# Da1yuqin/TCDiff

Hardware: AMD Instinct MI355X
Metric: sampled clips/sec (3 dancers x 150 frames, 1000 DDPM steps) (higher is better)
Workload: dtype bf16; 1 GPU; batch=16 clips/GPU, 3 dancers x 150 frames, 1000 DDPM steps (p_sample_loop, CFG w=2, cosine schedule), bf16, 1xMI355X; clips_per_gpu=16, ddpm_steps=1000

## Files before the change

include/tcdiff_hip.h:

```cpp
#ifndef TCDIFF_HIP_H
#define TCDIFF_HIP_H

#include <stdint.h>

#ifdef __cplusplus
extern "C" {
#endif

#ifndef __HIP__
typedef struct ihipStream_t* hipStream_t;
#endif

#define TCDIFF_OK 0
#define TCDIFF_ERR_ARG (-1)
#define TCDIFF_ERR_ALIGN (-2)
#define TCDIFF_ERR_LAUNCH (-3)
#define TCDIFF_ERR_UNSUPPORTED (-4)

#define TC_DTYPE_F32 0
#define TC_DTYPE_BF16 1
#define TC_DTYPE_BF16X3 2

#define TC_ACT_NONE 0
#define TC_ACT_RELU 1
// ... 246 lines not shown
} tcdiff_ct_desc;
int tcdiff_ct_desc_init(int dtype, tcdiff_ct_desc* d);
int tcdiff_cast_transpose_multi(int dtype, const tcdiff_ct_desc* descs_dev, int n_desc, int n_tiles, hipStream_t stream);

typedef struct tcdiff_ws_desc {
    const float* src;
    void* dst;
    long sn, sk;
    int N, K;
    int np_dst, p0, kst_dst, ks0;
} tcdiff_ws_desc;
int tcdiff_pack_row_streams(const tcdiff_ws_desc* descs_dev, int n_desc, int max_elems, hipStream_t stream);
int tcdiff_gemm_rows(const void* A, const void* A2, int split_n, const void* wstream, int M, int N, int K, int lda,
                     const tcdiff_tile_epi* epi, int mt, hipStream_t stream);

int tcdiff_gemm_splitk(int dtype, const void* A, const void* W, int M, int N, int K, int lda, int ldw, float* out,
                       int ldc, int splits, hipStream_t stream);

int tcdiff_gemm_tn(int dtype, const void* A, const void* B, int M, int N, int K, int lda, int ldb, float* out, int ldc,
                   int splits, hipStream_t stream);

#define TC_TN_MAX_PROB 16
typedef struct {
    const void* A; const void* B; float* out;
    int M, N, K, lda, ldb, ldc;
    int nk, unit0;
} tcdiff_tn_problem;
typedef struct {
    int n_prob, total_units, units_per_wg, kc;
    tcdiff_tn_problem p[TC_TN_MAX_PROB];
// ... 210 lines not shown
```

tcdiff_amd/_lib.py:

```python
import ctypes as C
import os

HERE = os.path.dirname(os.path.abspath(__file__))
LIB_PATH = os.environ.get("TCDIFF_LIB_PATH") or os.path.join(HERE, "libtcdiff_gfx950.so")

DT_F32, DT_BF16, DT_BF16X3 = 0, 1, 2
ACT_NONE, ACT_RELU, ACT_GELU, ACT_MISH, ACT_SILU = 0, 1, 2, 3, 4
EPI_STORE_T, EPI_STORE_F32, EPI_QKV_HEADS = 0, 1, 2
ROW_BIAS, ROW_LN_POST, ROW_FILM, ROW_RES, ROW_STORE_X, ROW_NEXT_LN, ROW_STORE_H, ROW_STORE_ROT = \
    1, 2, 4, 8, 16, 32, 64, 128
SAMPLER_DDPM, SAMPLER_DDIM = 0, 1
EXPORT_NORMAL, EXPORT_LONG = 0, 1
SAMPLER_ADVANCE = 0x100
CHAIN_A, CHAIN_B, CHAIN_B_LAST, CHAIN_FULL, CHAIN_FULL_LAST, CHAIN_FRONT = 0, 1, 2, 3, 4, 5

_vp, _i, _f, _l = C.c_void_p, C.c_int, C.c_float, C.c_long


class TileEpi(C.Structure):
    _fields_ = [("mode", _i), ("act", _i), ("scale_q", _f), ("bias", _vp), ("out", _vp), ("out_k", _vp),
                ("out_v", _vp), ("ldc", _i), ("L", _i), ("Lp", _i), ("H", _i), ("n_q", _i), ("n_k", _i),
                ("tok_off", _i), ("seq_off", _i), ("k_splits", _i), ("out2", _vp), ("ldc2", _i), ("act_src", _vp),
                ("ld_src", _i), ("act2", _i), ("drop_seed", _vp), ("drop_site", _i), ("drop_thr", C.c_uint32),
                ("drop_scale", _f), ("hgroup", _i), ("hgroup_stride", _l), ("small_m", _i)]
# ... 110 lines not shown
    "tcdiff_step_prologue": [_i, _vp, _vp],
    "tcdiff_sampler_update": [_i, _vp, _vp, _i, _vp, _vp, _vp, _vp, _i, _i, _i, _vp, _vp, _vp, C.c_uint64, _i, _vp],
    "tcdiff_window_couple": [_vp, _i, _i, _i, _vp],
    "tcdiff_window_couple_step": [_vp, _i, _i, _i, _vp, _vp, _vp],
    "tcdiff_sampler_constrain": [_i, _vp, _vp, _i, _vp, _vp, _i, _i, _i, _vp, _vp, _vp, C.c_uint64, _i, _vp],
    "tcdiff_ema_update": [_vp, _i, _f, _f, _vp],
    "tcdiff_cfg_combine": [_vp, _vp, _i, _f, _vp, _i, _i, _vp],
    "tcdiff_cast_transpose": [_i, _i, _vp, _i, _i, _i, _vp, _i, _i, _vp, _i, _i, _vp, _vp],
    "tcdiff_gemm_splitk": [_i, _vp, _vp, _i, _i, _i, _i, _i, _vp, _i, _i, _vp],
    "tcdiff_gemm_tn": [_i, _vp, _vp, _i, _i, _i, _i, _i, _vp, _i, _i, _vp],
    "tcdiff_gemm_tn_grouped": [_i, C.POINTER(TnProblem), _i, _vp],
    "tcdiff_ct_desc_init": [_i, C.POINTER(CtDesc)],
    "tcdiff_cast_transpose_multi": [_i, _vp, _i, _i, _vp],
    "tcdiff_pack_row_streams": [_vp, _i, _i, _vp],
    "tcdiff_gemm_rows": [_vp, _vp, _i, _vp, _i, _i, _i, _i, _vp, _i, _vp],
    "tcdiff_pos_drop": [_vp, _i, _i, _vp, _i, _vp, _i, C.c_uint32, _f, _vp],
    "tcdiff_act_drop": [_i, _i, _vp, _i, _vp, _i, _i, _i, _i, _vp, _i, C.c_uint32, _f, _vp],
    "tcdiff_act_drop_bwd": [_i, _i, _vp, _i, _vp, _i, _vp, _i, _i, _i, _vp, _i, C.c_uint32, _f, _vp],
    "tcdiff_row_fwd": [_i, C.POINTER(RowArgs), _vp],
    "tcdiff_row_bwd": [_i, C.POINTER(RowArgs), _vp],
    "tcdiff_row_param_reduce": [_vp, _i, _vp, _vp, _vp, _vp, _vp, _vp],
    "tcdiff_attention_train": [_i, _vp, _vp, _vp, _vp, _vp, _vp, _i, _i, _i, _i, _i, _i, _i, _vp, _i, C.c_uint32, _f, _vp],
    "tcdiff_attention_bwd": [_i, _vp, _vp, _vp, _vp, _vp, _vp, _vp, _vp, _vp, _i, _vp, _vp, _i, _i, _i, _i, _i, _i, _i, _i,
                             _f, _vp, _i, C.c_uint32, _f, _vp],
    "tcdiff_add_rows": [_vp, _i, _vp, _i, _vp, _i, _i, _i, _vp],
    "tcdiff_select_rows": [_vp, _vp, _vp, _vp, _i, _l, _vp],
    "tcdiff_select_rows_bwd": [_vp, _vp, _vp, _vp, _i, _l, _vp],
    "tcdiff_pool_bwd": [_vp, _vp, _vp, _i, _i, _i, _vp],
    "tcdiff_loss_total": [_vp, _i, _vp, _vp],
    "tcdiff_loss_terms_bwd": [_vp, _vp, _vp, _vp, _vp, _vp, _vp, _vp, _vp, _i, _i, _i, _i, _i, _vp],
# ... 71 lines not shown
```

tcdiff_amd/build.py:

```python
import os
import subprocess
import sys

HERE = os.path.dirname(os.path.abspath(__file__))
ROOT = os.path.dirname(HERE)
SRC = [os.path.join(HERE, "csrc", f) for f in ("gemm.hip", "attention.hip", "ops.hip", "chain.hip", "train.hip", "train_ops.hip",
                                               "attention_train.hip", "gemm_rows.hip", "chain_split.hip", "export.hip", "navigator.hip", "navigator_train.hip", "navigator_step.hip",
                                               "ingest.hip", "handoff.hip")]
HDR = sorted(os.path.join(HERE, "csrc", h) for h in os.listdir(os.path.join(HERE, "csrc")) if h.endswith(".h")) + \
    [os.path.join(ROOT, "include", "tcdiff_hip.h")]
LIB = os.path.join(HERE, "libtcdiff_gfx950.so")


def needs_build() -> bool:
    if not os.path.exists(LIB):
        return True
    t = os.path.getmtime(LIB)
    return any(os.path.getmtime(f) > t for f in SRC + HDR)


def build(force: bool = False, verbose: bool = True) -> str:
    if not force and not needs_build():
        return LIB
    hipcc = os.environ.get("HIPCC", "/opt/rocm/bin/hipcc")
# ... 24 lines not shown
```

tcdiff_amd/csrc/chain_core.h:

```cpp
#pragma once
#include "common.h"
#include "tcdiff_hip.h"

#define CH_FILM 0
#define CH_VEC 8192
#define CH_SCR 20480
#define CH_ABUF 28672
#define CH_H1C 94208
#define CH_ABUF2 94208
#define CH_STG7 159744
#define CH_SMEM 163840
#define CH_D 4
#define CH_STAGE 4096
#ifndef CH_D8
#define CH_D8 4
#endif
template <int NT> struct ChW {
    static constexpr int NW = 32 / NT;
    static constexpr int D = NT == 8 ? CH_D8 : CH_D;
    static constexpr int STAGE = 1024 * NT;
};

typedef const float* fptr;

// ... 447 lines not shown
            const int row = row0 + 8 * k;
            const u32x4 v = *reinterpret_cast<const u32x4*>(stg + row * 128 + ((ch ^ ((row >> 1) & 7)) << 4));
            if (m < M) *reinterpret_cast<u32x4*>(dst) = v;
            m += 8;
            tokf += 8;
            dst += 8 * 64 * dn;
            if (tokf >= Lf) {
                tokf -= Lf;
                dst += wrap;
            }
        }
    }
    }
}

#define CH_LOG2E 1.4426950408889634f
#ifndef CH_ATT_THR
#define CH_ATT_THR 5.0f
#endif

DEVINL float max3n(float a, float b, float c) { return __builtin_fmaximum_numf(__builtin_fmaximum_numf(a, b), c); }
DEVINL float lane_max8(const f32x4_t& a, const f32x4_t& b, float floor) {
    return max3n(max3n(max3n(max3n(a[0], a[1], a[2]), a[3], b[0]), b[1], b[2]), b[3], floor);
}

template <int MT>
DEVINL void store_qfrag(const f32x4_t (&acc)[4][MT], void* base, float scale, int lblk, int wave, int lane) {
    u32x4* dst = reinterpret_cast<u32x4*>(base) + ((long)(lblk * 8 + wave) * 8) * 64 + lane;
    scale *= CH_LOG2E;
#pragma unroll
// ... 62 lines not shown
```

tcdiff_amd/csrc/gemm_rows.hip:

```cpp
#include "chain_core.h"
#include "train_common.h"

struct RowsArgs {
    const char* A;
    const char* A2;
    const char* wstream;
    int split_n, n_stages, M, N, lda_bytes;
    tcdiff_tile_epi e;
};

DEVINL void unpack8(const u32x4& c, float (&v)[8]) {
#pragma unroll
    for (int i = 0; i < 4; ++i) {
        v[2 * i] = __builtin_bit_cast(float, c[i] << 16);
        v[2 * i + 1] = __builtin_bit_cast(float, c[i] & 0xFFFF0000u);
    }
}
DEVINL u32x4 pack8(const float (&v)[8]) {
    u32x4 c;
#pragma unroll
    for (int i = 0; i < 4; ++i) c[i] = pack_bf2(v[2 * i], v[2 * i + 1]);
    return c;
}

template <int MT, class F>
DEVINL void staged_rows(const f32x4_t (&acc)[4][MT], char* stg, int lane, F&& sink) {
    lane = fresh_v(lane);
    const int c = lane & 15, g = lane >> 4;
    const int row0 = lane >> 3, ch = lane & 7;
    constexpr int NH = MT == 4 ? 2 : 1, NML = MT == 1 ? 1 : 2;
#pragma unroll
    for (int hf = 0; hf < NH; ++hf) {
#pragma unroll
        for (int ml = 0; ml < NML; ++ml) {
            const int rl = 16 * ml + c;
#pragma unroll
            for (int nt = 0; nt < 4; ++nt) {
                const f32x4_t v = acc[nt][2 * hf + ml];
                uint2 pk;
                pk.x = pack_bf2(v[0], v[1]);
                pk.y = pack_bf2(v[2], v[3]);
                *reinterpret_cast<uint2*>(stg + rl * 128 + (((2 * nt + (g >> 1)) ^ ((rl >> 1) & 7)) << 4) + 8 * (g & 1)) = pk;
            }
        }
#pragma unroll
        for (int k = 0; k < 2 * NML; ++k) {
            const int row = row0 + 8 * k;
            const u32x4 v = *reinterpret_cast<const u32x4*>(stg + row * 128 + ((ch ^ ((row >> 1) & 7)) << 4));
            sink(32 * hf + row, ch, v);
        }
    }
}

template <int KST, int MT>
__global__ __launch_bounds__(512) void gemm_rows_kernel(RowsArgs a) {
    constexpr int BR = 16 * MT;
    extern __shared__ __attribute__((aligned(16))) char smem[];
    const int tid = threadIdx.x, lane = tid & 63;
    const int wave = __builtin_amdgcn_readfirstlane(tid >> 6);
    const int m0 = xcd_remap(blockIdx.x, gridDim.x) * BR;
    const int M = a.M;
    char* abuf = smem + CH_ABUF;
    char* abuf2 = smem + CH_ABUF2;
    const bool two = KST == 16 && a.A2 != nullptr;

    if (wave < 2 * MT) {
// ... 221 lines not shown
```

tcdiff_amd/csrc/ops.hip:

```cpp
#include "common.h"
#include "tcdiff_hip.h"

DEVINL long kf_index(int key, int d) {
    const int kt = key >> 5, k32 = key & 31, d32 = d & 31;
    const int g = (d32 & 15) >> 2, jj = 4 * (d32 >> 4) + (d32 & 3);
    return ((long)((kt * 2 + (k32 >> 4)) * 2 + (d >> 5)) * 64 + g * 16 + (k32 & 15)) * 8 + jj;
}
DEVINL long vf_index(int key, int d) {
    const int kt = key >> 5, k32 = key & 31;
    const int g = (k32 & 15) >> 2, jj = 4 * (k32 >> 4) + (k32 & 3);
    return ((long)(kt * 4 + (d >> 4)) * 64 + g * 16 + (d & 15)) * 8 + jj;
}

template <class P>
__global__ __launch_bounds__(256) void ln_rot_kernel(const float* __restrict__ x, int rows, const float* __restrict__ g,
                                                     const float* __restrict__ b, float eps, void* __restrict__ hout,
                                                     void* __restrict__ rout, float* __restrict__ y32,
                                                     const float* __restrict__ rope, int pos_mod, int pos_base) {
    typedef typename P::elem_t T;
    const int lane = threadIdx.x & 63;
    const int row = blockIdx.x * 4 + (threadIdx.x >> 6);
    if (row >= rows) return;
    const float* xr = x + (long)row * 512;
    f32x4_t v[2];
// ... 256 lines not shown
    hipLaunchKernelGGL(step_end_kernel, dim3(1), dim3(64), 0, stream, counter);
    TC_CHECK_LAUNCH();
    return TC_OK;
}

template <class P>
__global__ __launch_bounds__(256) void step_prologue_kernel(tcdiff_step_prologue_args a) {
    typedef typename P::elem_t E;
    int* counter = a.counter;
    const int step = counter[3];
    const int t = a.tseq[step];
    const bool do_x = a.parts == 0 || (a.parts & TC_PROLOGUE_X), do_c = a.parts == 0 || (a.parts & TC_PROLOGUE_COND);
    const long n_film = (long)a.n_seq * 512;
    const long n_kv = do_c ? (long)a.NL * a.n_kv * 2 * 1024 : 0;
    const bool x8 = std::is_same<P, MmaBF16>::value && a.ld_xin % 8 == 0;
    const long n_x = (a.x && do_x) ? (x8 ? (long)a.rows * (a.ld_xin / 8) : (long)a.rows * a.ld_xin) : 0;
    const long q_tab = (a.film_tab && do_c) ? (long)a.n_seq * (a.nfilm / 4) : 0;
    const long total = n_film + n_kv + n_x + q_tab;
    for (long i = (long)blockIdx.x * blockDim.x + threadIdx.x; i < total; i += (long)gridDim.x * blockDim.x) {
        if (i >= n_film + n_kv + n_x) {
            const long k = i - (n_film + n_kv + n_x);
            const int q4 = a.nfilm / 4;
            const int seq = (int)(k / q4), c4 = (int)(k % q4);
            const int j = seq < a.n_unc ? 0 : seq - a.n_unc + 1;
            reinterpret_cast<f32x4_t*>(a.film_out)[(long)seq * q4 + c4] =
                reinterpret_cast<const f32x4_t*>(a.film_tab)[((long)t * a.film_rows + j) * q4 + c4];
        } else if (i < n_film) {
            const int c = (int)(i & 511);
            if (c == 0 && do_x) a.tidx[i >> 9] = t;
            if (!a.film_tab && do_c) store_T<P>((E*)a.film_in, i, mish_f(a.t_base[(long)t * 512 + c] + a.hidden[i]));
        } else if (i < n_film + n_kv) {
// ... 21 lines not shown
                const u32x4 pk = {pack_bf2(v[0], v[1]), pack_bf2(v[2], v[3]), pack_bf2(v[4], v[5]), pack_bf2(v[6], v[7])};
                *reinterpret_cast<u32x4*>(reinterpret_cast<uint16_t*>(a.xin) + (long)r * a.ld_xin + c0) = pk;
            } else {
                const int r = (int)(k / a.ld_xin), c = (int)(k % a.ld_xin);
                store_T<P>((E*)a.xin, k, c < a.nfeat ? a.x[(long)r * a.nfeat + c] : 0.0f);
            }
        }
    }
    if (do_x && blockIdx.x == 0 && threadIdx.x == 0) counter[0] = step;
}

extern "C" int tcdiff_step_prologue(int dtype, const tcdiff_step_prologue_args* a, hipStream_t stream) {
    if (!a || !a->counter || !a->tseq || !a->tidx || !a->t_base || !a->hidden || !a->film_in || !a->tab ||
        a->n_seq <= 0 || a->NL <= 0 || a->n_kv <= 0 || a->H * 64 != 512 || (!a->Kc && !a->Kf) || (!a->Kc != !a->Vc) ||
        (!a->Kf != !a->Vf) || a->tok0 + 1 >= a->Lp || (a->Kf && a->tok0 + 2 > 32 * a->nkt) ||
        (a->x && (!a->xin || a->rows <= 0 || a->ld_xin < a->nfeat)))
        return TC_ERR_ARG;
    if (a->Kf && dtype != TC_DTYPE_BF16) return TC_ERR_ARG;
    if (a->film_tab && (!a->film_out || a->film_rows <= 0 || a->nfilm <= 0 || a->nfilm % 4 || a->n_unc < 0 ||
                        a->n_seq - a->n_unc + 1 > a->film_rows ||
                        ((reinterpret_cast<uintptr_t>(a->film_tab) | reinterpret_cast<uintptr_t>(a->film_out)) & 15)))
        return TC_ERR_ARG;
    if (a->parts < 0 || a->parts > (TC_PROLOGUE_X | TC_PROLOGUE_COND)) return TC_ERR_ARG;
    const bool do_x = a->parts == 0 || (a->parts & TC_PROLOGUE_X), do_c = a->parts == 0 || (a->parts & TC_PROLOGUE_COND);
    const bool x8 = dtype == TC_DTYPE_BF16 && a->ld_xin % 8 == 0;
    if (x8 && a->x && (reinterpret_cast<uintptr_t>(a->xin) & 15)) return TC_ERR_ALIGN;
    const long total = (long)a->n_seq * 512 + (do_c ? (long)a->NL * a->n_kv * 2048 : 0) +
                       ((a->x && do_x) ? (x8 ? (long)a->rows * (a->ld_xin / 8) : (long)a->rows * a->ld_xin) : 0) +
                       ((a->film_tab && do_c) ? (long)a->n_seq * (a->nfilm / 4) : 0);
    const unsigned grid = (unsigned)std::min<long>((total + 255) / 256, 2048);
    if (dtype == TC_DTYPE_BF16)
        hipLaunchKernelGGL(step_prologue_kernel<MmaBF16>, dim3(grid), dim3(256), 0, stream, *a);
    else if (dtype == TC_DTYPE_F32)
        hipLaunchKernelGGL(step_prologue_kernel<MmaF32>, dim3(grid), dim3(256), 0, stream, *a);
    else if (dtype == TC_DTYPE_BF16X3 && a->ld_xin % 4 == 0)
        hipLaunchKernelGGL(step_prologue_kernel<MmaBF16x3>, dim3(grid), dim3(256), 0, stream, *a);
    else
        return TC_ERR_ARG;
    TC_CHECK_LAUNCH();
    return TC_OK;
}

DEVINL void philox_round(uint32_t (&c)[4], uint32_t k0, uint32_t k1) {
// ... 263 lines not shown
```

tcdiff_amd/diffusion.py:

```python
from __future__ import annotations

import copy
import os
from typing import Callable, Optional

import numpy as np
import torch
import torch.nn as nn

from . import _lib as L
from . import kernels as K


def cosine_beta_schedule(n_timestep: int, cosine_s: float = 8e-3) -> np.ndarray:
    steps = torch.arange(n_timestep + 1, dtype=torch.float64) / n_timestep + cosine_s
    ac = torch.cos(steps / (1 + cosine_s) * np.pi / 2).pow(2)
    ac = ac / ac[0]
    return np.clip((1 - ac[1:] / ac[:-1]).numpy(), a_min=0, a_max=0.999)


def make_beta_schedule(schedule, n_timestep, linear_start=1e-4, linear_end=2e-2, cosine_s=8e-3) -> np.ndarray:
    if schedule == "cosine":
        return cosine_beta_schedule(n_timestep, cosine_s)
    if schedule == "linear":
# ... 233 lines not shown
            t = tseq[i]
            branches = 1 if w_eff[i] == 1.0 else 2
            if unroll > 1 and i >= run_until:
                j = i
                while j < n and (1 if w_eff[j] == 1.0 else 2) == branches:
                    j += 1
                run_until, run_u = j, self._steps_per_graph(j - i, unroll)
            u = run_u if (unroll > 1 and i + run_u <= run_until) else 1
            if step_noise is not None:
                st["eps"].copy_(step_noise(int(t), (B, Lq, nf)).reshape(B * Lq, nf))
            if q_noise is not None:
                st["qeps"].copy_(q_noise(int(t), (B, Lq, nf)).reshape(B * Lq, nf))
            ckey = None if constrain is None else (constrain["kind"], q_noise is not None, mask_rows, constrain.get("params") is not None)
            split = eng._split_job(branches * B)
            form = (split, split and eng._merge12(Lq), split and eng.front and os.environ.get("TCDIFF_SPLIT_FRONT", "1") != "0",
                    os.environ.get("TCDIFF_FORK_PROLOGUE", "0") == "1")
            gkey = (mode, branches, step_noise is not None, traj is not None, clip_offset, B, gen, id(self.model), ckey, couple, u, form)
            if not use_graph:
                step(branches)
            elif gkey in graphs:
                graphs[gkey].replay()
            elif ("warm", gkey) not in graphs:
                for _ in range(u):
                    step(branches)
                graphs[("warm", gkey)] = True
            else:
                for k in [k for k in graphs if is_step_key(k) and k[7] == id(self.model) and k[6] != gen]:
                    del graphs[k]
                live = [k for k in graphs if is_step_key(k)]
                for k in live[:max(0, len(live) - 15)]:
                    del graphs[k]
# ... 355 lines not shown
```

tcdiff_amd/engine.py:

```python
from __future__ import annotations

import math
import os
from typing import Dict, Optional

import torch

from . import _lib as L
from . import kernels as K

MERGE12_MAX_L = 512
NL_FILM = 3


class DenoiserEngine:
    def __init__(self, cfg: dict, device: torch.device, compute: str = "bf16"):
        L.load()
        if device.type != "cuda":
            raise L.TcdiffError("DenoiserEngine needs a HIP device (cuda:N); there is no CPU fallback")
        self.cfg = dict(cfg)
        self.dev = device
        self.dt = K.dtype_id(compute)
        self.T = K.TORCH_DT[self.dt]
        self.kt = K.k_tile(self.dt)
# ... 18 lines not shown
        self._sampler_state = None
        self._side, self._forked = None, False
        self._xcur = 0
        self.act = int(cfg.get("act", L.ACT_GELU))
        self.abs_pos = bool(cfg.get("abs_pos", False))
        self.use_chain = self.dt == L.DT_BF16 and os.environ.get("TCDIFF_CHAIN", "1") != "0" and self.ff == 1024 \
            and self.H == 8 and self.act == L.ACT_GELU and not self.abs_pos
        self.use_full = self.use_chain and os.environ.get("TCDIFF_CHAIN", "2") == "2"
        self.nkt = (self.S + 2 + 31) // 32
        self.fold_in = self.dt == L.DT_BF16 and os.environ.get("TCDIFF_FOLD_IN", "1") != "0"
        self.kin = K.round_up(self.dn * self.nf, 64)
        self.fold_out = self.use_chain and os.environ.get("TCDIFF_FOLD_OUT", "1") != "0"
        self.front = self.use_full and os.environ.get("TCDIFF_FRONT", "1") != "0" and self.S >= 8
        self.fuse_sa = self.use_full and self.dt == L.DT_BF16 and os.environ.get("TCDIFF_FUSE_SA", "1") == "1"
        self.chain_nw = int(os.environ.get("TCDIFF_CHAIN_NW", "8"))
        if self.chain_nw not in (4, 8):
            raise L.TcdiffError("TCDIFF_CHAIN_NW must be 8 or 4")
        self.reset_graphs()

    def reset_graphs(self):
        self.graphs = {}
        self.graph_warm = set()
        self.generation = getattr(self, "generation", 0) + 1

    def sampler_state(self, n_steps: int, rows: int, nfeat: int):
        st = self._sampler_state
        if st is None or st["x"].shape != (rows, nfeat) or st["cap"] < n_steps:
            cap = max(4096, n_steps)
            dev = self.dev
            st = dict(cap=cap,
# ... 14 lines not shown
        out = torch.zeros(n, kp, device=self.dev, dtype=self.T)
        out[:, :k] = w.to(device=self.dev, dtype=self.T)
        if self.dt == L.DT_BF16X3:
            return K.to_x3(out)
        return out.contiguous()

    _PI = (0, 3, 1, 2)

    @staticmethod
    def _stages_n512(W: torch.Tensor, nw: int = 8) -> torch.Tensor:
        K_, NT = W.shape[1], 32 // nw
        w6 = W.reshape(nw, NT, 16, K_ // 32, 4, 8)[:, :, :, :, list(DenoiserEngine._PI), :]
        return w6.permute(0, 3, 1, 4, 2, 5).reshape(nw, K_ // 32, 512 * NT)

    @staticmethod
    def _stages_ff1(W1: torch.Tensor, nw: int = 8) -> torch.Tensor:
        NH = 16 // nw
        w8 = W1.reshape(4, nw, NH, 16, 8, 2, 4, 8)[:, :, :, :, :, :, list(DenoiserEngine._PI), :]
        return w8.permute(0, 1, 4, 5, 2, 6, 3, 7).reshape(4, nw, 8, 1024 * NH)

    @staticmethod
    def _stages_ff2(W2: torch.Tensor, nw: int = 8) -> torch.Tensor:
        NT = 32 // nw
        w7 = W2.reshape(nw, NT, 16, 4, 8, 4, 8)[:, :, :, :, :, list(DenoiserEngine._PI), :]
        return w7.permute(3, 0, 4, 1, 5, 2, 6).reshape(4, nw, 8, 512 * NT)

    @staticmethod
    def _ffn_order(f1, f2):
        return [f for c in range(4) for f in (f1[c], f2[c])]

    def _build_chain_streams(self):
        w = self.w
        nw = self.chain_nw
        n512 = self._stages_n512
        if self.front:
            qkv = w["l0.qkv.w"]
            tail = [n512(qkv[0:512], nw), n512(qkv[512:1024], nw), n512(qkv[1024:1536], nw)]
            w["front"] = torch.stack([torch.cat([n512(w["f3.w"][512 * d:512 * d + 512], nw)] + tail, 1)
                                      for d in range(self.dn)]).contiguous()
        for l in range(self.NL):
            p = f"l{l}."
            if l + 1 < self.NL or not self.fold_out:
                W3 = w[p + "l3.w"]
            else:
                W3f = self.sd_f32(f"seqTransDecoder.stack.{l}.linear3.weight")
                b3 = self.sd_f32(f"seqTransDecoder.stack.{l}.linear3.bias")
                Wf, bf = self.sd_f32("final_layer.weight"), self.sd_f32("final_layer.bias")
                Wo = torch.zeros(512, 512, device=self.dev, dtype=torch.float32)
                Wo[:self.nf] = Wf @ W3f
# ... 99 lines not shown
        if self.use_chain:
            self._build_chain_streams()
        self.sd_f32 = None
        self.weights_version = version
        self.tables_key = None
        self.reset_graphs()

    def plan(self, B: int):
        if B == self.plan_B:
            return
        dev, T = self.dev, self.T
        z = lambda *s, dtype=T: torch.zeros(*s, device=dev, dtype=dtype)
        Lq, S, H, NL = self.Lseq, self.S, self.H, self.NL
        R = 2 * B * Lq
        b = {}
        b["xin"] = z(B * S, self.kin) if self.fold_in else z(B * Lq, 192)
        b["xp"] = z(B * Lq, 512)
        b["f1"], b["f2"] = z(B * S, 1024), z(B * S, 1024)
        b["xs"] = z(B * Lq, 512, dtype=torch.float32)
        b["h"], b["rot"], b["O"] = z(R, 512), z(R, 512), z(R, 512)
        b["Q"], b["K"] = z(2 * B, H, self.Lp, 64), z(2 * B, H, self.Lp, 64)
        b["V"] = z(2 * B, H, self.Lp, 64)
        b["xa"] = z(R, 512, dtype=torch.float32)
        b["h1"] = z(R, 1024)
        b["out"] = z(R, 152, dtype=torch.float32)
        b["film"] = z(2 * B, NL * NL_FILM * 1024, dtype=torch.float32)
        b["film_in"] = z(2 * B, 512)
        b["Kc"] = z(NL, 2 * B, H, self.Lpc, 64)
        b["Vc"] = z(NL, 2 * B, H, self.Lpc, 64)
        if self.use_full:
            b["Kf"] = z(NL, 2 * B, H, self.nkt * 2048)
            b["Vf"] = z(NL, 2 * B, H, self.nkt * 2048)
        if self.fuse_sa:
            self.skt = (Lq + 31) // 32
            self.n_cu = torch.cuda.get_device_properties(dev).multi_processor_count
            b["Qf"] = z(2 * B * ((Lq + 15) // 16), 8, 4, 2, 64, 8)
            b["sKf"], b["sVf"] = z(2, 2 * B, H, self.skt * 2048), z(2, 2 * B, H, self.skt * 2048)
            if self._split_rows(2 * B, Lq):
                nblk = 2 * B * ((Lq + 15) // 16)
                b["xb"] = z(R, 512, dtype=torch.float32)
                b["P0"], b["P1"] = z(nblk, 4, 16, 512, dtype=torch.float32), z(nblk, 4, 16, 512, dtype=torch.float32)
        b["hidden_all"] = z(2 * B, 512, dtype=torch.float32)
        b["tidx"] = torch.zeros(2 * B, device=dev, dtype=torch.int32)
        b["cin"] = z(B * S, K.round_up(2 * self.cfg["cond_dim"], 64))
        b["c1"] = z(B * S, K.round_up(self.cfg["cond_dim"], 64))
        b["tok"] = z(B * S, 512, dtype=torch.float32)
        b["mh"], b["mrot"], b["mO"] = z(B * S, 512), z(B * S, 512), z(B * S, 512)
        b["mQ"], b["mK"] = z(B, H, self.Lps, 64), z(B, H, self.Lps, 64)
        b["mV"] = z(B, H, self.Lps, 64)
        b["mh1"] = z(B * S, 1024)
        b["pool"] = z(B, 512, dtype=torch.float32)
        b["pool_h"], b["pool_h2"] = z(B, 512), z(B, 512)
        b["hidden"] = z(B, 512, dtype=torch.float32)
# ... 115 lines not shown
            return token_rows // self.dn, self.dn * self.nf, self.kin
        return token_rows, self.nf, 192

    def step_prologue(self, st: dict, n_rows_seq: int, x: torch.Tensor, rows: int):
        dt, w, b = self.dt, self.w, self.b
        full = self.use_full
        nfilm = self.NL * NL_FILM * 1024
        tab = getattr(self, "film_tab", None)
        if tab is not None and tab.shape[1] * 2 - 2 != n_rows_seq:
            tab = None
        extra = {} if tab is None else dict(film_tab=tab, film_out=b["film"], film_rows=tab.shape[1], nfilm=nfilm,
                                            n_unc=n_rows_seq // 2)
        args = (dt, st["counter"], st["rows"], b["tidx"], self.t_base, b["hidden_all"], b["film_in"],
                n_rows_seq, self.kv_tab, self.n_t, None if full else b["Kc"], None if full else b["Vc"],
                b["Kf"] if full else None, b["Vf"] if full else None, self.NL, b["Kc"].shape[1], self.H,
                self.Lpc, self.nkt if full else 0, self.S, x, b["xin"], *self._xin_shape(rows))
        if tab is not None and self.use_chain and self.front and os.environ.get("TCDIFF_FORK_PROLOGUE", "0") == "1":
            K.step_prologue(*args, parts=L.PROLOGUE_X, **extra)
            main = torch.cuda.current_stream()
            if self._side is None:
                self._side = torch.cuda.Stream(device=self.dev)
            self._side.wait_stream(main)
            with torch.cuda.stream(self._side):
                K.step_prologue(*args, parts=L.PROLOGUE_COND, **extra)
            self._forked = True
            return
        K.step_prologue(*args, **extra)
        if tab is None:
            K.gemm_tile(dt, b["film_in"], w["film.w"], n_rows_seq, nfilm, 512, bias=w["film.b"], mode=L.EPI_STORE_F32,
                        out=b["film"], ldc=nfilm)

    def network(self, x: torch.Tensor, B: int, branches: int, kv_slot0: int, n_shared: int, film_row0: int,
                x_ready: bool = False):
        dt, w, b = self.dt, self.w, self.b
        Lq, S, H, dn, NL = self.Lseq, self.S, self.H, self.dn, self.NL
        Rs, R = B * Lq, branches * B * Lq
        nseq = branches * B
        fld = NL * NL_FILM * 1024
        film0 = b["film"][film_row0:]
        rope = w["rope"]
        if not x_ready:
            K.convert_pad(dt, x, b["xin"], *self._xin_shape(Rs))
        sm = self._split_job(nseq)
        if self.fold_in:
            K.gemm_tile(dt, b["xin"], w["f1in.w"], B * S, 1024, self.kin, bias=w["f1in.b"], act=L.ACT_RELU, out=b["f1"],
                        ldc=1024, small_m=sm)
        else:
            K.gemm_tile(dt, b["xin"], w["in.w"], Rs, 512, 192, bias=w["in.b"], out=b["xp"], ldc=512, small_m=sm)
            K.gemm_tile(dt, b["xp"], w["f1.w"], B * S, 1024, 512 * dn, bias=w["f1.b"], act=L.ACT_RELU, out=b["f1"],
                        ldc=1024, small_m=sm)
        K.gemm_tile(dt, b["f1"], w["f2.w"], B * S, 1024, 1024, bias=w["f2.b"], act=L.ACT_RELU, out=b["f2"], ldc=1024, small_m=sm)
        self._frag_front = self.front and self._split_job(nseq) and os.environ.get("TCDIFF_SPLIT_FRONT", "1") != "0"
        if self._frag_front:
            K.gemm_tile(dt, b["f2"], w["f3.w"], B * S, 512 * dn, 1024, bias=w["f3.b"], mode=L.EPI_STORE_F32, out=b["xs"],
                        ldc=512 * dn, small_m=True)
            K.chain(L.CHAIN_FRONT, Rs, Lq, None, w["front"][0], split_part=0, xres=b["xs"], nn_g=w["l0.norm1.g"],
                    nn_b=w["l0.norm1.b"], nn_eps=1e-5, rope=w["rope_cb"], qf_out=b["Qf"], kf_out=b["sKf"][0], vf_out=b["sVf"][0],
                    out_nkt=self.skt, scale_q=0.125, H=H)
        elif self.front:
            K.chain(L.CHAIN_FRONT, B * S, Lq, b["f2"], w["front"], b3=w["f3.b"], nn_g=w["l0.norm1.g"],
                    nn_b=w["l0.norm1.b"], nn_eps=1e-5, rope=w["rope_cb"], xout=b["xs"], q_out=b["Q"], k_out=b["K"],
                    v_out=b["V"], scale_q=0.125, Lp=self.Lp, H=H, dn=dn)
        elif self.abs_pos:
            K.gemm_rowln(dt, b["f2"], w["f3.w"], B * S, 1024, bias=w["f3.b"], xout=b["xs"], Lseq=Lq,
                         flags=L.ROW_BIAS | L.ROW_STORE_X, out_mul=dn, out_add=0, groups=dn)
            K.add_rows(b["xs"], 512, b["pe_x"], 512, b["xs"], 512, Rs, 512)
# ... 39 lines not shown
                         bias=w[p + "ff2.b"], film=film0[:, (l * 3 + 2) * 1024:], film_ld=fld, xres=b["xa"], Lseq=Lq,
                         nln_g=w[p + "norm4.g"], nln_b=w[p + "norm4.b"], nln_eps=1e-5, hout=b["h"])
            if l + 1 < NL:
                n1 = f"l{l + 1}.norm1."
                K.gemm_rowln(dt, b["h"], w[p + "l3.w"], R, 512, bias=w[p + "l3.b"], xout=b["xa"], Lseq=Lq,
                             flags=L.ROW_BIAS | L.ROW_STORE_X | L.ROW_NEXT_LN | L.ROW_STORE_H | L.ROW_STORE_ROT,
                             nln_g=w[n1 + "g"], nln_b=w[n1 + "b"], nln_eps=1e-5, hout=b["h"], rout=b["rot"], rope=rope)
            else:
                K.gemm_rowln(dt, b["h"], w[p + "l3.w"], R, 512, bias=w[p + "l3.b"], Lseq=Lq,
                             flags=L.ROW_BIAS | L.ROW_STORE_H, hout=b["h"])
        if self.fold_out:
            return b["out"]
        K.gemm_tile(dt, b["h"], w["fin.w"], R, self.nf, 512, bias=w["fin.b"], mode=L.EPI_STORE_F32, out=b["out"], ldc=152)
        return b["out"]

    def _split_job(self, nseq: int) -> bool:
        return bool(self.use_full and self.fuse_sa and self.chain_nw == 8 and "xb" in self.b and self._split_rows(nseq, self.Lseq))

    @staticmethod
    def _merge12(Lq: int) -> bool:
        v = os.environ.get("TCDIFF_SPLIT_MERGE", "")
        return v == "1" or (v != "0" and Lq <= MERGE12_MAX_L)

    def _split_rows(self, nseq: int, Lq: int) -> bool:
        if os.environ.get("TCDIFF_SPLIT", "1") == "0" or self.chain_nw != 8 or Lq < 16:
            return False
        return 4 * nseq * ((Lq + 15) // 16) <= self.n_cu

    def _layer_chained(self, l: int, B: int, branches: int, Kc0, Vc0, film0, fld: int, n_shared: int, kv_slot0: int):
        dt, w, b = self.dt, self.w, self.b
# ... 66 lines not shown
```

tcdiff_amd/kernels.py:

```python
import ctypes as C

import torch

from . import _lib as L

TORCH_DT = {L.DT_F32: torch.float32, L.DT_BF16: torch.bfloat16, L.DT_BF16X3: torch.float32}


def dtype_id(name_or_dtype) -> int:
    if isinstance(name_or_dtype, str) and name_or_dtype == "bf16x3":
        return L.DT_BF16X3
    if name_or_dtype in ("bf16", torch.bfloat16, L.DT_BF16):
        return L.DT_BF16
    if name_or_dtype in ("f32", "fp32", torch.float32, L.DT_F32):
        return L.DT_F32
    if name_or_dtype == L.DT_BF16X3 and not isinstance(name_or_dtype, bool):
        return L.DT_BF16X3
    raise ValueError(f"unsupported compute dtype {name_or_dtype!r} (bf16, f32 or bf16x3)")


def k_tile(dt: int) -> int:
    return 64 if dt == L.DT_BF16 else 32


# ... 46 lines not shown

def gemm_rows_ok(dt, N, K) -> bool:
    return dt == L.DT_BF16 and K in (512, 1024) and N > 0 and N % 512 == 0


def gemm_rows(A, wstream, M, N, K, *, lda=None, A2=None, split_n=0, mode=L.EPI_STORE_T, bias=None, out=None, ldc=0,
              out_k=None, out_v=None, scale_q=1.0, Lseq=0, Lp=0, H=0, n_q=0, n_k=0, out2=None, ldc2=0, act_src=None, ld_src=0,
              act2=L.ACT_NONE, seed=None, site=0, thr=0, drop_scale=1.0, mt=0):
    if tuple(wstream.shape) != (8, (N // 512) * (K // 32), 2048) or not wstream.is_contiguous():
        raise L.TcdiffError(f"weight stream of a [{N}, {K}] matrix must be contiguous [8, {(N // 512) * (K // 32)}, 2048], got "
                            f"{tuple(wstream.shape)}")
    e = L.TileEpi(mode, L.ACT_NONE, scale_q, _p(bias), _p(out), _p(out_k), _p(out_v), ldc, Lseq, Lp, H, n_q, n_k, 0, 0, 0,
                  _p(out2), ldc2, _p(act_src), ld_src, act2, _p(seed), site, thr, drop_scale, 0, 0)
    rc = L.load().tcdiff_gemm_rows(_p(A), _p(A2), split_n, _p(wstream), M, N, K, lda if lda else K, C.byref(e), mt, stream())
    L.check(rc, "tcdiff_gemm_rows")


def ws_table(entries, device):
    n = len(entries)
    arr = (L.WsDesc * n)()
    mx = 0
    for d, e in zip(arr, entries):
        N, K_ = e["N"], e["K"]
        if e["src"].dtype != torch.float32 or N % 512 or K_ % 32:
            raise L.TcdiffError("pack_row_streams takes fp32 sources with N % 512 == 0 and K % 32 == 0")
        npd, p0, kd, ks0 = e.get("np_dst", N // 512), e.get("p0", 0), e.get("kst_dst", K_ // 32), e.get("ks0", 0)
        if p0 + N // 512 > npd or ks0 + K_ // 32 > kd:
            raise L.TcdiffError("pack_row_streams: the piece does not fit the stream")
        if e["dst"].numel() != 8 * npd * kd * 2048 or e["dst"].element_size() != 2 or not e["dst"].is_contiguous():
            raise L.TcdiffError("pack_row_streams: dst must be a contiguous 2-byte tensor of [8, np_dst * kst_dst, 2048]")
# ... 399 lines not shown
```

Baseline: 14.77 clips/s.

## Fuse input convert, MLP layer 1 and layer 2 into one row-streaming kernel

Adds a fusion_rows kernel that loads fp32 input rows, casts them to bf16 in LDS, and runs the first 1024-wide ReLU layer with the hidden kept in shared memory. It then runs the second 1024x1024 ReLU layer from a pre-packed weight stream and writes bf16 output. This replaces the separate convert_pad launch, two gemm_tile launches and the f1 round trip through memory in the non-split front path. The xin buffer is dropped when it is no longer needed, and the prologue tolerates a null xin. The risk is lower parallelism: each block covers 16 rows and streams all the weights, so grids with few rows may use the CUs poorly.

```diff
diff --git a/include/tcdiff_hip.h b/include/tcdiff_hip.h
--- a/include/tcdiff_hip.h
+++ b/include/tcdiff_hip.h
@@ -284,6 +284,9 @@
 int tcdiff_gemm_rows(const void* A, const void* A2, int split_n, const void* wstream, int M, int N, int K, int lda,
                      const tcdiff_tile_epi* epi, int mt, hipStream_t stream);
 
+int tcdiff_fusion_rows(const float* x, int M, int kx, const void* wstream, int k1, const float* b1, const float* b2, void* out,
+                       int ldc, hipStream_t stream);
+
 int tcdiff_gemm_splitk(int dtype, const void* A, const void* W, int M, int N, int K, int lda, int ldw, float* out,
                        int ldc, int splits, hipStream_t stream);
 
diff --git a/tcdiff_amd/_lib.py b/tcdiff_amd/_lib.py
--- a/tcdiff_amd/_lib.py
+++ b/tcdiff_amd/_lib.py
@@ -148,6 +148,7 @@
     "tcdiff_cast_transpose_multi": [_i, _vp, _i, _i, _vp],
     "tcdiff_pack_row_streams": [_vp, _i, _i, _vp],
     "tcdiff_gemm_rows": [_vp, _vp, _i, _vp, _i, _i, _i, _i, _vp, _i, _vp],
+    "tcdiff_fusion_rows": [_vp, _i, _i, _vp, _i, _vp, _vp, _vp, _i, _vp],
     "tcdiff_pos_drop": [_vp, _i, _i, _vp, _i, _vp, _i, C.c_uint32, _f, _vp],
     "tcdiff_act_drop": [_i, _i, _vp, _i, _vp, _i, _i, _i, _i, _vp, _i, C.c_uint32, _f, _vp],
     "tcdiff_act_drop_bwd": [_i, _i, _vp, _i, _vp, _i, _vp, _i, _i, _i, _vp, _i, C.c_uint32, _f, _vp],
diff --git a/tcdiff_amd/build.py b/tcdiff_amd/build.py
--- a/tcdiff_amd/build.py
+++ b/tcdiff_amd/build.py
@@ -5,7 +5,7 @@
 HERE = os.path.dirname(os.path.abspath(__file__))
 ROOT = os.path.dirname(HERE)
 SRC = [os.path.join(HERE, "csrc", f) for f in ("gemm.hip", "attention.hip", "ops.hip", "chain.hip", "train.hip", "train_ops.hip",
-                                               "attention_train.hip", "gemm_rows.hip", "chain_split.hip", "export.hip", "navigator.hip", "navigator_train.hip", "navigator_step.hip",
+                                               "attention_train.hip", "gemm_rows.hip", "fusion_rows.hip", "chain_split.hip", "export.hip", "navigator.hip", "navigator_train.hip", "navigator_step.hip",
                                                "ingest.hip", "handoff.hip")]
 HDR = sorted(os.path.join(HERE, "csrc", h) for h in os.listdir(os.path.join(HERE, "csrc")) if h.endswith(".h")) + \
     [os.path.join(ROOT, "include", "tcdiff_hip.h")]
diff --git a/tcdiff_amd/csrc/chain_core.h b/tcdiff_amd/csrc/chain_core.h
--- a/tcdiff_amd/csrc/chain_core.h
+++ b/tcdiff_amd/csrc/chain_core.h
@@ -485,6 +485,35 @@
     }
 }
 
+template <int MT, class F>
+DEVINL void staged_rows(const f32x4_t (&acc)[4][MT], char* stg, int lane, F&& sink) {
+    lane = fresh_v(lane);
+    const int c = lane & 15, g = lane >> 4;
+    const int row0 = lane >> 3, ch = lane & 7;
+    constexpr int NH = MT == 4 ? 2 : 1, NML = MT == 1 ? 1 : 2;
+#pragma unroll
+    for (int hf = 0; hf < NH; ++hf) {
+#pragma unroll
+        for (int ml = 0; ml < NML; ++ml) {
+            const int rl = 16 * ml + c;
+#pragma unroll
+            for (int nt = 0; nt < 4; ++nt) {
+                const f32x4_t v = acc[nt][2 * hf + ml];
+                uint2 pk;
+                pk.x = pack_bf2(v[0], v[1]);
+                pk.y = pack_bf2(v[2], v[3]);
+                *reinterpret_cast<uint2*>(stg + rl * 128 + (((2 * nt + (g >> 1)) ^ ((rl >> 1) & 7)) << 4) + 8 * (g & 1)) = pk;
+            }
+        }
+#pragma unroll
+        for (int k = 0; k < 2 * NML; ++k) {
+            const int row = row0 + 8 * k;
+            const u32x4 v = *reinterpret_cast<const u32x4*>(stg + row * 128 + ((ch ^ ((row >> 1) & 7)) << 4));
+            sink(32 * hf + row, ch, v);
+        }
+    }
+}
+
 #define CH_LOG2E 1.4426950408889634f
 #ifndef CH_ATT_THR
 #define CH_ATT_THR 5.0f
diff --git a/tcdiff_amd/csrc/fusion_rows.hip b/tcdiff_amd/csrc/fusion_rows.hip
--- /dev/null
+++ b/tcdiff_amd/csrc/fusion_rows.hip
@@ -0,0 +1,131 @@
+#include "chain_core.h"
+
+struct FusionArgs {
+    const float* x;
+    const char* wstream;
+    const float *b1, *b2;
+    uint16_t* out;
+    int M, kx, n_stages, ldc;
+};
+
+#define FR_XOFF 2048
+
+template <int KST1>
+__global__ __launch_bounds__(512) void fusion_rows_kernel(FusionArgs a) {
+    extern __shared__ __attribute__((aligned(16))) char smem[];
+    const int tid = threadIdx.x, lane = tid & 63;
+    const int wave = __builtin_amdgcn_readfirstlane(tid >> 6);
+    const int m0 = blockIdx.x * 16;
+    const int M = a.M, kx = a.kx;
+    char* hbuf = smem + CH_ABUF;
+
+    constexpr int NCH = 16 * KST1 * 4;
+    constexpr int NPASS = (NCH + 511) / 512;
+    float xv[NPASS][8];
+#pragma unroll
+    for (int i = 0; i < NPASS; ++i) {
+        const int q = tid + 512 * i;
+        const int row = q / (KST1 * 4), k0 = (q % (KST1 * 4)) * 8;
+        const bool live = q < NCH && m0 + row < M;
+        const float* src = a.x + (long)(m0 + row) * kx + k0;
+#pragma unroll
+        for (int j = 0; j < 8; ++j) xv[i][j] = (live && k0 + j < kx) ? src[j] : 0.0f;
+    }
+    WStream ws;
+    ws.rsrc = __builtin_amdgcn_make_buffer_rsrc(const_cast<char*>(a.wstream) + (long)wave * a.n_stages * CH_STAGE, 0,
+                                                a.n_stages * CH_STAGE, 0x00020000);
+    ws.voff = (unsigned)lane * 16u;
+    ws.pos = 0;
+    ws.last = (unsigned)a.n_stages - 1;
+#pragma unroll
+    for (int i = 0; i < CH_D; ++i) ws_load(ws, i, (unsigned)i);
+#pragma unroll
+    for (int i = 0; i < NPASS; ++i) {
+        const int q = tid + 512 * i;
+        if (q < NCH) {
+            const int row = q / (KST1 * 4), ch = q % (KST1 * 4);
+            const u32x4 pk = {pack_bf2(xv[i][0], xv[i][1]), pack_bf2(xv[i][2], xv[i][3]), pack_bf2(xv[i][4], xv[i][5]),
+                              pack_bf2(xv[i][6], xv[i][7])};
+            *reinterpret_cast<u32x4*>(hbuf + FR_XOFF + (ch >> 3) * 8192 + tile_off(row, ch & 7)) = pk;
+        }
+    }
+    __syncthreads();
+
+#pragma unroll 1
+    for (int p = 0; p < 2; ++p) {
+        f32x4_t acc[4][1];
+        zero(acc);
+        phase_n512<KST1, false, 1>(acc, hbuf + FR_XOFF, ws, lane);
+        const int ln = fresh_v(lane);
+        const int g = ln >> 4;
+        const float* bias = a.b1 + 512 * p + 64 * wave + 4 * g;
+        char* dst = hbuf + (8 * p + wave) * 8192;
+#pragma unroll
+        for (int nt = 0; nt < 4; ++nt) {
+            const f32x4_t v = acc[nt][0] + ld4(bias + 16 * nt);
+            uint2 pk;
+            pk.x = pack_bf2(fmaxf(v[0], 0.0f), fmaxf(v[1], 0.0f));
+            pk.y = pack_bf2(fmaxf(v[2], 0.0f), fmaxf(v[3], 0.0f));
+            *reinterpret_cast<uint2*>(dst + act_wr_off(ln, nt)) = pk;
+        }
+    }
+    __syncthreads();
+
+    char* stg = stage_area(smem, wave);
+#pragma unroll 1
+    for (int p = 0; p < 2; ++p) {
+        f32x4_t acc[4][1];
+        zero(acc);
+        phase_n512<32, false, 1>(acc, hbuf, ws, lane);
+        const int ln = fresh_v(lane);
+        const int g = ln >> 4;
+        const int col0 = 512 * p + 64 * wave;
+        const float* bias = a.b2 + col0 + 4 * g;
+#pragma unroll
+        for (int nt = 0; nt < 4; ++nt) {
+            const f32x4_t v = acc[nt][0] + ld4(bias + 16 * nt);
+            acc[nt][0] = f32x4_t{fmaxf(v[0], 0.0f), fmaxf(v[1], 0.0f), fmaxf(v[2], 0.0f), fmaxf(v[3], 0.0f)};
+        }
+        staged_rows<1>(acc, stg, lane, [&](int row, int ch, const u32x4& val) {
+            const int m = m0 + row;
+            if (m < M) *reinterpret_cast<u32x4*>(a.out + (long)m * a.ldc + col0 + 8 * ch) = val;
+        });
+    }
+}
+
+static bool fr_al16(const void* p) { return (reinterpret_cast<uintptr_t>(p) & 15) == 0; }
+
+extern "C" int tcdiff_fusion_rows(const float* x, int M, int kx, const void* wstream, int k1, const float* b1, const float* b2,
+                                  void* out, int ldc, hipStream_t stream) {
+    if (!x || !wstream || !b1 || !b2 || !out || M <= 0 || kx <= 0) return TC_ERR_ARG;
+    if (k1 != 256 && k1 != 384 && k1 != 512) return TC_ERR_UNSUPPORTED;
+    if (kx > k1 || ldc < 1024) return TC_ERR_ARG;
+    if (ldc % 8 || !fr_al16(wstream) || !fr_al16(b1) || !fr_al16(b2) || !fr_al16(out)) return TC_ERR_ALIGN;
+    static tc_dev_state dev_state;
+    const int n_cu = tc_device_once(dev_state, [](int) {
+        const void* fns[3] = {reinterpret_cast<const void*>(fusion_rows_kernel<8>), reinterpret_cast<const void*>(fusion_rows_kernel<12>),
+                              reinterpret_cast<const void*>(fusion_rows_kernel<16>)};
+        for (const void* f : fns) {
+            hipError_t er = hipFuncSetAttribute(f, hipFuncAttributeMaxDynamicSharedMemorySize, CH_SMEM);
+            if (er != hipSuccess) return er;
+        }
+        return hipSuccess;
+    });
+    if (n_cu < 0) return n_cu;
+    FusionArgs a;
+    a.x = x;
+    a.wstream = reinterpret_cast<const char*>(wstream);
+    a.b1 = b1;
+    a.b2 = b2;
+    a.out = reinterpret_cast<uint16_t*>(out);
+    a.M = M;
+    a.kx = kx;
+    a.n_stages = 2 * (k1 / 32) + 64;
+    a.ldc = ldc;
+    const dim3 grid((M + 15) / 16);
+    if (k1 == 256) hipLaunchKernelGGL(fusion_rows_kernel<8>, grid, dim3(512), CH_SMEM, stream, a);
+    else if (k1 == 384) hipLaunchKernelGGL(fusion_rows_kernel<12>, grid, dim3(512), CH_SMEM, stream, a);
+    else hipLaunchKernelGGL(fusion_rows_kernel<16>, grid, dim3(512), CH_SMEM, stream, a);
+    TC_CHECK_LAUNCH();
+    return TC_OK;
+}
diff --git a/tcdiff_amd/csrc/gemm_rows.hip b/tcdiff_amd/csrc/gemm_rows.hip
--- a/tcdiff_amd/csrc/gemm_rows.hip
+++ b/tcdiff_amd/csrc/gemm_rows.hip
@@ -21,35 +21,6 @@
 #pragma unroll
     for (int i = 0; i < 4; ++i) c[i] = pack_bf2(v[2 * i], v[2 * i + 1]);
     return c;
-}
-
-template <int MT, class F>
-DEVINL void staged_rows(const f32x4_t (&acc)[4][MT], char* stg, int lane, F&& sink) {
-    lane = fresh_v(lane);
-    const int c = lane & 15, g = lane >> 4;
-    const int row0 = lane >> 3, ch = lane & 7;
-    constexpr int NH = MT == 4 ? 2 : 1, NML = MT == 1 ? 1 : 2;
-#pragma unroll
-    for (int hf = 0; hf < NH; ++hf) {
-#pragma unroll
-        for (int ml = 0; ml < NML; ++ml) {
-            const int rl = 16 * ml + c;
-#pragma unroll
-            for (int nt = 0; nt < 4; ++nt) {
-                const f32x4_t v = acc[nt][2 * hf + ml];
-                uint2 pk;
-                pk.x = pack_bf2(v[0], v[1]);
-                pk.y = pack_bf2(v[2], v[3]);
-                *reinterpret_cast<uint2*>(stg + rl * 128 + (((2 * nt + (g >> 1)) ^ ((rl >> 1) & 7)) << 4) + 8 * (g & 1)) = pk;
-            }
-        }
-#pragma unroll
-        for (int k = 0; k < 2 * NML; ++k) {
-            const int row = row0 + 8 * k;
-            const u32x4 v = *reinterpret_cast<const u32x4*>(stg + row * 128 + ((ch ^ ((row >> 1) & 7)) << 4));
-            sink(32 * hf + row, ch, v);
-        }
-    }
 }
 
 template <int KST, int MT>
diff --git a/tcdiff_amd/csrc/ops.hip b/tcdiff_amd/csrc/ops.hip
--- a/tcdiff_amd/csrc/ops.hip
+++ b/tcdiff_amd/csrc/ops.hip
@@ -294,7 +294,7 @@
     const long n_film = (long)a.n_seq * 512;
     const long n_kv = do_c ? (long)a.NL * a.n_kv * 2 * 1024 : 0;
     const bool x8 = std::is_same<P, MmaBF16>::value && a.ld_xin % 8 == 0;
-    const long n_x = (a.x && do_x) ? (x8 ? (long)a.rows * (a.ld_xin / 8) : (long)a.rows * a.ld_xin) : 0;
+    const long n_x = (a.x && a.xin && do_x) ? (x8 ? (long)a.rows * (a.ld_xin / 8) : (long)a.rows * a.ld_xin) : 0;
     const long q_tab = (a.film_tab && do_c) ? (long)a.n_seq * (a.nfilm / 4) : 0;
     const long total = n_film + n_kv + n_x + q_tab;
     for (long i = (long)blockIdx.x * blockDim.x + threadIdx.x; i < total; i += (long)gridDim.x * blockDim.x) {
@@ -346,7 +346,7 @@
     if (!a || !a->counter || !a->tseq || !a->tidx || !a->t_base || !a->hidden || !a->film_in || !a->tab ||
         a->n_seq <= 0 || a->NL <= 0 || a->n_kv <= 0 || a->H * 64 != 512 || (!a->Kc && !a->Kf) || (!a->Kc != !a->Vc) ||
         (!a->Kf != !a->Vf) || a->tok0 + 1 >= a->Lp || (a->Kf && a->tok0 + 2 > 32 * a->nkt) ||
-        (a->x && (!a->xin || a->rows <= 0 || a->ld_xin < a->nfeat)))
+        (a->x && a->xin && (a->rows <= 0 || a->ld_xin < a->nfeat)))
         return TC_ERR_ARG;
     if (a->Kf && dtype != TC_DTYPE_BF16) return TC_ERR_ARG;
     if (a->film_tab && (!a->film_out || a->film_rows <= 0 || a->nfilm <= 0 || a->nfilm % 4 || a->n_unc < 0 ||
@@ -356,9 +356,9 @@
     if (a->parts < 0 || a->parts > (TC_PROLOGUE_X | TC_PROLOGUE_COND)) return TC_ERR_ARG;
     const bool do_x = a->parts == 0 || (a->parts & TC_PROLOGUE_X), do_c = a->parts == 0 || (a->parts & TC_PROLOGUE_COND);
     const bool x8 = dtype == TC_DTYPE_BF16 && a->ld_xin % 8 == 0;
-    if (x8 && a->x && (reinterpret_cast<uintptr_t>(a->xin) & 15)) return TC_ERR_ALIGN;
+    if (x8 && a->x && a->xin && (reinterpret_cast<uintptr_t>(a->xin) & 15)) return TC_ERR_ALIGN;
     const long total = (long)a->n_seq * 512 + (do_c ? (long)a->NL * a->n_kv * 2048 : 0) +
-                       ((a->x && do_x) ? (x8 ? (long)a->rows * (a->ld_xin / 8) : (long)a->rows * a->ld_xin) : 0) +
+                       ((a->x && a->xin && do_x) ? (x8 ? (long)a->rows * (a->ld_xin / 8) : (long)a->rows * a->ld_xin) : 0) +
                        ((a->film_tab && do_c) ? (long)a->n_seq * (a->nfilm / 4) : 0);
     const unsigned grid = (unsigned)std::min<long>((total + 255) / 256, 2048);
     if (dtype == TC_DTYPE_BF16)
diff --git a/tcdiff_amd/diffusion.py b/tcdiff_amd/diffusion.py
--- a/tcdiff_amd/diffusion.py
+++ b/tcdiff_amd/diffusion.py
@@ -271,7 +271,7 @@
             ckey = None if constrain is None else (constrain["kind"], q_noise is not None, mask_rows, constrain.get("params") is not None)
             split = eng._split_job(branches * B)
             form = (split, split and eng._merge12(Lq), split and eng.front and os.environ.get("TCDIFF_SPLIT_FRONT", "1") != "0",
-                    os.environ.get("TCDIFF_FORK_PROLOGUE", "0") == "1")
+                    os.environ.get("TCDIFF_FORK_PROLOGUE", "0") == "1", eng.use_fused_mlp(branches * B))
             gkey = (mode, branches, step_noise is not None, traj is not None, clip_offset, B, gen, id(self.model), ckey, couple, u, form)
             if not use_graph:
                 step(branches)
diff --git a/tcdiff_amd/engine.py b/tcdiff_amd/engine.py
--- a/tcdiff_amd/engine.py
+++ b/tcdiff_amd/engine.py
@@ -56,6 +56,8 @@
         self.front = self.use_full and os.environ.get("TCDIFF_FRONT", "1") != "0" and self.S >= 8
         self.fuse_sa = self.use_full and self.dt == L.DT_BF16 and os.environ.get("TCDIFF_FUSE_SA", "1") == "1"
         self.chain_nw = int(os.environ.get("TCDIFF_CHAIN_NW", "8"))
+        self.fused_mlp = self.fold_in and self.front and K.fusion_k1(self.dn * self.nf) > 0 and \
+            os.environ.get("TCDIFF_FUSED_MLP", "1") != "0"
         if self.chain_nw not in (4, 8):
             raise L.TcdiffError("TCDIFF_CHAIN_NW must be 8 or 4")
         self.reset_graphs()
@@ -100,6 +102,16 @@
         return w6.permute(0, 3, 1, 4, 2, 5).reshape(nw, K_ // 32, 512 * NT)
 
     @staticmethod
+    def _fusion_stream(W1: torch.Tensor, W2: torch.Tensor) -> torch.Tensor:
+        k1 = K.fusion_k1(W1.shape[1])
+        if k1 == 0 or W1.shape[0] != 1024 or tuple(W2.shape) != (1024, 1024):
+            raise L.TcdiffError(f"_fusion_stream: W1 {tuple(W1.shape)}, W2 {tuple(W2.shape)}")
+        W1p = torch.zeros(1024, k1, device=W1.device, dtype=W1.dtype)
+        W1p[:, :W1.shape[1]] = W1
+        n512 = DenoiserEngine._stages_n512
+        return torch.cat([n512(W1p[:512]), n512(W1p[512:]), n512(W2[:512]), n512(W2[512:])], 1).contiguous()
+
+    @staticmethod
     def _stages_ff1(W1: torch.Tensor, nw: int = 8) -> torch.Tensor:
         NH = 16 // nw
         w8 = W1.reshape(4, nw, NH, 16, 8, 2, 4, 8)[:, :, :, :, :, :, list(DenoiserEngine._PI), :]
@@ -119,6 +131,8 @@
         w = self.w
         nw = self.chain_nw
         n512 = self._stages_n512
+        if self.fused_mlp:
+            w["fmlp"] = self._fusion_stream(w["f1in.w"], w["f2.w"])
         if self.front:
             qkv = w["l0.qkv.w"]
             tail = [n512(qkv[0:512], nw), n512(qkv[512:1024], nw), n512(qkv[1024:1536], nw)]
@@ -248,7 +262,11 @@
         Lq, S, H, NL = self.Lseq, self.S, self.H, self.NL
         R = 2 * B * Lq
         b = {}
-        b["xin"] = z(B * S, self.kin) if self.fold_in else z(B * Lq, 192)
+        if self.fuse_sa:
+            self.n_cu = torch.cuda.get_device_properties(dev).multi_processor_count
+        self._small_plan = bool(self.fuse_sa and self._split_rows(2 * B, Lq))
+        if not self.fused_mlp or self._small_plan:
+            b["xin"] = z(B * S, self.kin) if self.fold_in else z(B * Lq, 192)
         b["xp"] = z(B * Lq, 512)
         b["f1"], b["f2"] = z(B * S, 1024), z(B * S, 1024)
         b["xs"] = z(B * Lq, 512, dtype=torch.float32)
@@ -267,10 +285,9 @@
             b["Vf"] = z(NL, 2 * B, H, self.nkt * 2048)
         if self.fuse_sa:
             self.skt = (Lq + 31) // 32
-            self.n_cu = torch.cuda.get_device_properties(dev).multi_processor_count
             b["Qf"] = z(2 * B * ((Lq + 15) // 16), 8, 4, 2, 64, 8)
             b["sKf"], b["sVf"] = z(2, 2 * B, H, self.skt * 2048), z(2, 2 * B, H, self.skt * 2048)
-            if self._split_rows(2 * B, Lq):
+            if self._small_plan:
                 nblk = 2 * B * ((Lq + 15) // 16)
                 b["xb"] = z(R, 512, dtype=torch.float32)
                 b["P0"], b["P1"] = z(nblk, 4, 16, 512, dtype=torch.float32), z(nblk, 4, 16, 512, dtype=torch.float32)
@@ -416,7 +433,7 @@
         args = (dt, st["counter"], st["rows"], b["tidx"], self.t_base, b["hidden_all"], b["film_in"],
                 n_rows_seq, self.kv_tab, self.n_t, None if full else b["Kc"], None if full else b["Vc"],
                 b["Kf"] if full else None, b["Vf"] if full else None, self.NL, b["Kc"].shape[1], self.H,
-                self.Lpc, self.nkt if full else 0, self.S, x, b["xin"], *self._xin_shape(rows))
+                self.Lpc, self.nkt if full else 0, self.S, x, b.get("xin"), *self._xin_shape(rows))
         if tab is not None and self.use_chain and self.front and os.environ.get("TCDIFF_FORK_PROLOGUE", "0") == "1":
             K.step_prologue(*args, parts=L.PROLOGUE_X, **extra)
             main = torch.cuda.current_stream()
@@ -441,17 +458,21 @@
         fld = NL * NL_FILM * 1024
         film0 = b["film"][film_row0:]
         rope = w["rope"]
-        if not x_ready:
+        sm = self._split_job(nseq)
+        fused = self.use_fused_mlp(nseq)
+        if not x_ready and not fused:
             K.convert_pad(dt, x, b["xin"], *self._xin_shape(Rs))
-        sm = self._split_job(nseq)
-        if self.fold_in:
+        if fused:
+            K.fusion_rows(x, B * S, dn * self.nf, w["fmlp"], w["f1in.b"], w["f2.b"], b["f2"], 1024)
+        elif self.fold_in:
             K.gemm_tile(dt, b["xin"], w["f1in.w"], B * S, 1024, self.kin, bias=w["f1in.b"], act=L.ACT_RELU, out=b["f1"],
                         ldc=1024, small_m=sm)
         else:
             K.gemm_tile(dt, b["xin"], w["in.w"], Rs, 512, 192, bias=w["in.b"], out=b["xp"], ldc=512, small_m=sm)
             K.gemm_tile(dt, b["xp"], w["f1.w"], B * S, 1024, 512 * dn, bias=w["f1.b"], act=L.ACT_RELU, out=b["f1"],
                         ldc=1024, small_m=sm)
-        K.gemm_tile(dt, b["f1"], w["f2.w"], B * S, 1024, 1024, bias=w["f2.b"], act=L.ACT_RELU, out=b["f2"], ldc=1024, small_m=sm)
+        if not fused:
+            K.gemm_tile(dt, b["f1"], w["f2.w"], B * S, 1024, 1024, bias=w["f2.b"], act=L.ACT_RELU, out=b["f2"], ldc=1024, small_m=sm)
         self._frag_front = self.front and self._split_job(nseq) and os.environ.get("TCDIFF_SPLIT_FRONT", "1") != "0"
         if self._frag_front:
             K.gemm_tile(dt, b["f2"], w["f3.w"], B * S, 512 * dn, 1024, bias=w["f3.b"], mode=L.EPI_STORE_F32, out=b["xs"],
@@ -521,6 +542,9 @@
         K.gemm_tile(dt, b["h"], w["fin.w"], R, self.nf, 512, bias=w["fin.b"], mode=L.EPI_STORE_F32, out=b["out"], ldc=152)
         return b["out"]
 
+    def use_fused_mlp(self, nseq: int) -> bool:
+        return self.fused_mlp and not self._split_job(nseq)
+
     def _split_job(self, nseq: int) -> bool:
         return bool(self.use_full and self.fuse_sa and self.chain_nw == 8 and "xb" in self.b and self._split_rows(nseq, self.Lseq))
 
diff --git a/tcdiff_amd/kernels.py b/tcdiff_amd/kernels.py
--- a/tcdiff_amd/kernels.py
+++ b/tcdiff_amd/kernels.py
@@ -84,6 +84,23 @@
                   _p(out2), ldc2, _p(act_src), ld_src, act2, _p(seed), site, thr, drop_scale, 0, 0)
     rc = L.load().tcdiff_gemm_rows(_p(A), _p(A2), split_n, _p(wstream), M, N, K, lda if lda else K, C.byref(e), mt, stream())
     L.check(rc, "tcdiff_gemm_rows")
+
+
+def fusion_k1(kx: int) -> int:
+    k1 = max(256, round_up(kx, 128))
+    return k1 if 0 < kx and k1 <= 512 else 0
+
+
+def fusion_rows(x, M, kx, wstream, b1, b2, out, ldc=1024):
+    k1 = fusion_k1(kx)
+    if k1 == 0 or tuple(wstream.shape) != (8, 2 * (k1 // 32) + 64, 2048) or not wstream.is_contiguous() or \
+            wstream.dtype != torch.bfloat16:
+        raise L.TcdiffError(f"fusion_rows: kx = {kx} needs a contiguous bf16 stream [8, {2 * (k1 // 32) + 64}, 2048], got "
+                            f"{tuple(wstream.shape)}")
+    if x.dtype != torch.float32 or not x.is_contiguous() or x.numel() < M * kx or b1.numel() < 1024 or b2.numel() < 1024 or \
+            out.dtype != torch.bfloat16 or out.numel() < (M - 1) * ldc + 1024:
+        raise L.TcdiffError("fusion_rows: x must be contiguous fp32 [M, kx], the biases 1024 floats, out bf16 [M, ldc]")
+    L.check(L.load().tcdiff_fusion_rows(_p(x), M, kx, _p(wstream), k1, _p(b1), _p(b2), _p(out), ldc, stream()), "tcdiff_fusion_rows")
 
 
 def ws_table(entries, device):
```

Result: no change. 14.77 clips/s (median of 4 runs) (+0.0%).
